# Thefefe/orbit

Measured on NVIDIA B200. Metric: Gmeshlets culled/s (C2: 10k entities / 2M meshlets, 1920x1080, two-pass occlusion, steady-state frame), higher is better.
Workload: dtype f32

## Files before the change

### orbit_b200/csrc/meshlet_cull.cu

```cuda
#include "params.cuh"

namespace orbit {

constexpr int kMcWarps = 8;
constexpr int kMcThreads = kMcWarps * 32;
constexpr int kMvStride = 20;
constexpr uint32_t kNone = 0xFFFFFFFFu;

struct ItemTest {
    Sphere s;
    bool pre_visible;
};

template <int kProj>
__device__ __forceinline__ ItemTest test_item(const OrbitCullInfo& ci, const float4 c0, const float4 c1, const float4 c2, const float4 c3,
                                              const float scale, const float cx, const float cy, const float cz, const float r_model,
                                              const uint32_t cone) {
    ItemTest out;
    float px = add(add(add(mul(c0.x, cx), mul(c1.x, cy)), mul(c2.x, cz)), c3.x);
    float py = add(add(add(mul(c0.y, cx), mul(c1.y, cy)), mul(c2.y, cz)), c3.y);
    float pz = add(add(add(mul(c0.z, cx), mul(c1.z, cy)), mul(c2.z, cz)), c3.z);
    const float pw = add(add(add(mul(c0.w, cx), mul(c1.w, cy)), mul(c2.w, cz)), c3.w);
    if (pw != 1.0f) { px = fdiv(px, pw); py = fdiv(py, pw); pz = fdiv(pz, pw); }
    Sphere& s = out.s;
    s.x = px; s.y = py; s.z = pz;
    s.r_model = r_model; s.s = scale;
    s.r = mul(s.r_model, scale);
    const float nr = -s.r;
    bool visible = true;
    const uint32_t n = ci.cull_plane_count;
    if (n == 5u) {
#pragma unroll
        for (uint32_t i = 0; i < 5u; ++i) {
            const float d = add(dot3(ci.cull_planes[i][0], ci.cull_planes[i][1], ci.cull_planes[i][2], px, py, pz), ci.cull_planes[i][3]);
            visible = visible && (d > nr);
        }
    } else {
#pragma unroll 1
        for (uint32_t i = 0; i < n; ++i) {
            const float d = add(dot3(ci.cull_planes[i][0], ci.cull_planes[i][1], ci.cull_planes[i][2], px, py, pz), ci.cull_planes[i][3]);
            visible = visible && (d > nr);
        }
    }
    {
        const float K = 0.007874015718698502f;
        const float kx = mul((float)(int)(int8_t)(cone & 0xFFu), K);
        const float ky = mul((float)(int)(int8_t)((cone >> 8) & 0xFFu), K);
        const float kz = mul((float)(int)(int8_t)((cone >> 16) & 0xFFu), K);
        const float cutoff = mul((float)((int)cone >> 24), K);
        const float axx = add(add(add(mul(c0.x, kx), mul(c1.x, ky)), mul(c2.x, kz)), mul(c3.x, 0.0f));
        const float axy = add(add(add(mul(c0.y, kx), mul(c1.y, ky)), mul(c2.y, kz)), mul(c3.y, 0.0f));
        const float axz = add(add(add(mul(c0.z, kx), mul(c1.z, ky)), mul(c2.z, kz)), mul(c3.z, 0.0f));
        const uint32_t proj = kProj >= 0 ? (uint32_t)kProj : ci.projection_type;
        if (proj == 0u) {
            const float lhs = dot3(px, py, pz, axx, axy, axz);
            const float len = fsqrt(dot3(px, py, pz, px, py, pz));
            visible = visible && !(lhs >= fma_(cutoff, len, s.r));
        } else if (proj == 1u) {
            const float camx = sub(px, 0.0f), camy = sub(py, 0.0f), camz = sub(pz, -1.0f);
            const float qx = sub(px, camx), qy = sub(py, camy), qz = sub(pz, camz);
            const float lhs = dot3(qx, qy, qz, axx, axy, axz);
            const float len = fsqrt(dot3(qx, qy, qz, qx, qy, qz));
            visible = visible && !(lhs >= fma_(cutoff, len, s.r));
        }
    }
    out.pre_visible = visible;
    return out;
}

__device__ __forceinline__ bool draw_rule(const OrbitCullInfo& ci, const MeshletCullParams& p, bool visible, bool vib, bool pass2,
                                          uint32_t packed) {
    if (!visible) return false;
    const uint32_t material_index = packed & 0xFFFFu;
    const uint32_t alpha = __ldg(reinterpret_cast<const uint32_t*>(
        p.materials + (size_t)material_index * ORBIT_MATERIAL_STRIDE_BYTES + ORBIT_MATERIAL_ALPHA_MODE_OFFSET));
    bool should_draw = (shl1(alpha) & ci.alpha_mode_flags) != 0u;
    if (pass2 && (shl1(alpha) & ci.noskip_alpha_mode) == 0u) should_draw = !vib;
    return should_draw;
}

__device__ __forceinline__ void store_command(uint32_t* __restrict__ dst, uint32_t vertex_offset, uint32_t data_offset, uint32_t packed,
                                              uint32_t entity, uint32_t meshlet_index) {
    dst[0] = (packed >> 24) * 3u;
    dst[1] = 1u;
    dst[2] = (data_offset + ((packed >> 16) & 0xFFu)) * 4u;
    dst[3] = data_offset;
    dst[4] = entity;
    dst[5] = vertex_offset;
    dst[6] = meshlet_index;
}

constexpr uint32_t kMaxChunks = 2048u;
__device__ __forceinline__ uint32_t chunk_shift_of(uint32_t nrec) {
    const uint32_t per = (nrec + kMaxChunks - 1u) / kMaxChunks;
    const uint32_t sh = per <= 1u ? 0u : 32u - (uint32_t)__clz((int)(per - 1u));
    return max(5u, sh);
}

__device__ __forceinline__ uint32_t smem_addr(const void* p) { return (uint32_t)__cvta_generic_to_shared(p); }
__device__ __forceinline__ void cp_async_16_stream(uint32_t dst, const void* src, uint64_t policy) {
    asm volatile("cp.async.cg.shared.global.L2::cache_hint [%0], [%1], 16, %2;" ::"r"(dst), "l"(src), "l"(policy) : "memory");
}
__device__ __forceinline__ void cp_async_16(uint32_t dst, const void* src) {
    asm volatile("cp.async.cg.shared.global [%0], [%1], 16;" ::"r"(dst), "l"(src) : "memory");
}
__device__ __forceinline__ void cp_async_4(uint32_t dst, const void* src) {
    asm volatile("cp.async.ca.shared.global [%0], [%1], 4;" ::"r"(dst), "l"(src) : "memory");
}
__device__ __forceinline__ void cp_async_commit() { asm volatile("cp.async.commit_group;" ::: "memory"); }
__device__ __forceinline__ void cp_async_wait_all() { asm volatile("cp.async.wait_group 0;" ::: "memory"); }
__device__ __forceinline__ uint64_t l2_evict_first_policy() {
    uint64_t pol;
    asm volatile("createpolicy.fractional.L2::evict_first.b64 %0, 1.0;" : "=l"(pol));
    return pol;
}
__device__ __forceinline__ void sts32(uint32_t addr, uint32_t v) { asm volatile("st.shared.u32 [%0], %1;" ::"r"(addr), "r"(v) : "memory"); }
__device__ __forceinline__ uint32_t lds32(uint32_t addr) { uint32_t v; asm volatile("ld.shared.u32 %0, [%1];" : "=r"(v) : "r"(addr) : "memory"); return v; }
__device__ __forceinline__ uint4 lds128(uint32_t addr) {
    uint4 v;
    asm volatile("ld.shared.v4.u32 {%0, %1, %2, %3}, [%4];" : "=r"(v.x), "=r"(v.y), "=r"(v.z), "=r"(v.w) : "r"(addr) : "memory");
    return v;
}

struct PkConsts { float2 one, mone; };
ORBIT_DEV float2 pk(float a, float b) { return make_float2(a, b); }
ORBIT_DEV float2 pmul(float2 a, float2 b) { return __fmul2_rn(a, b); }
ORBIT_DEV float2 pmuls(float2 a, float s) { return __fmul2_rn(a, make_float2(s, s)); }
ORBIT_DEV float2 pfma(float2 a, float2 b, float2 c) { return __ffma2_rn(a, b, c); }
ORBIT_DEV float2 padd(const PkConsts& k, float2 a, float2 b) { return __ffma2_rn(a, k.one, b); }
ORBIT_DEV float2 psub(const PkConsts& k, float2 a, float2 b) { return __ffma2_rn(b, k.mone, a); }
ORBIT_DEV float2 pneg(const PkConsts& k, float2 a) { return __fmul2_rn(a, k.mone); }
ORBIT_DEV float2 pdot3(const PkConsts& k, float2 ax, float2 ay, float2 az, float2 bx, float2 by, float2 bz) {
    return padd(k, padd(k, pmul(ax, bx), pmul(ay, by)), pmul(az, bz));
}
ORBIT_DEV float2 psqrt(float2 a) { return make_float2(fsqrt(a.x), fsqrt(a.y)); }
ORBIT_DEV float2 pdiv(float2 a, float2 b) { return make_float2(fdiv(a.x, b.x), fdiv(a.y, b.y)); }

struct ItemXY { float2 pxy; float pz, r; bool pre_visible; };
ORBIT_DEV float2 lo2(const float4 v) { return make_float2(v.x, v.y); }
ORBIT_DEV float2 hi2(const float4 v) { return make_float2(v.z, v.w); }

template <int kProj>
__device__ __forceinline__ ItemXY test_item_xy(const OrbitCullInfo& ci, const MeshletCullParams& p, const PkConsts& k, const float4 c0, const float4 c1,
                                              const float4 c2, const float4 c3, const float scale, const float cx, const float cy, const float cz,
                                              const float r_model, const uint32_t cone) {
    ItemXY out;
    float2 pxy = padd(k, padd(k, padd(k, pmuls(lo2(c0), cx), pmuls(lo2(c1), cy)), pmuls(lo2(c2), cz)), lo2(c3));
    const float2 pzw = padd(k, padd(k, padd(k, pmuls(hi2(c0), cx), pmuls(hi2(c1), cy)), pmuls(hi2(c2), cz)), hi2(c3));
    float pz = pzw.x;
    if (pzw.y != 1.0f) { pxy.x = fdiv(pxy.x, pzw.y); pxy.y = fdiv(pxy.y, pzw.y); pz = fdiv(pz, pzw.y); }
    const float r = mul(r_model, scale);
    out.pxy = pxy; out.pz = pz; out.r = r;
// ... 63 lines not shown
        const float2 nrc1 = pmul(nr, c1), rc1 = pmul(r, c1);
        const float2 sxc0 = pmul(sx, c0), sxc1 = pmul(sx, c1), syd0 = pmul(sy, d0), syc1 = pmul(sy, c1);
        const float2 minx0 = padd(k, sxc0, nrc1), minx1 = padd(k, pmul(r, c0), sxc1);
        const float2 maxx0 = padd(k, sxc0, rc1), maxx1 = padd(k, pmul(nr, c0), sxc1);
        const float2 miny0 = padd(k, syd0, nrc1), miny1 = padd(k, pmul(r, d0), syc1);
        const float2 maxy0 = padd(k, syd0, rc1), maxy1 = padd(k, pmul(nr, d0), syc1);
        const float2 a0 = pmuls(pdiv(minx0, minx1), P00), a1 = pmuls(pdiv(miny0, miny1), P11);
        const float2 a2 = pmuls(pdiv(maxx0, maxx1), P00), a3 = pmuls(pdiv(maxy0, maxy1), P11);
        const float2 h = pk(0.5f, 0.5f), nh = pk(-0.5f, -0.5f);
        ax = pfma(a0, h, h); ay = pfma(a3, nh, h);
        az = pfma(a2, h, h); aw = pfma(a1, nh, h);
        depth = pdiv(pk(ci.z_near, ci.z_near), pfma(pneg(k, r_model), s, zp));
    } else if (proj == 1u) {
        const float sr = ci.p00_or_width_recip_x2;
        const float2 ctrx = pmuls(x, sr), ctry = pmuls(y, sr);
        const float2 box = pmuls(r, sr);
        const float2 one = pk(1.0f, 1.0f), mone = pk(-1.0f, -1.0f);
        float2 b0 = pfma(box, mone, ctrx), b1 = pfma(box, mone, ctry);
        float2 b2 = pfma(box, one, ctrx), b3 = pfma(box, one, ctry);
        b0 = pk(fminf(fmaxf(b0.x, -1.0f), 1.0f), fminf(fmaxf(b0.y, -1.0f), 1.0f));
        b1 = pk(fminf(fmaxf(b1.x, -1.0f), 1.0f), fminf(fmaxf(b1.y, -1.0f), 1.0f));
        b2 = pk(fminf(fmaxf(b2.x, -1.0f), 1.0f), fminf(fmaxf(b2.y, -1.0f), 1.0f));
        b3 = pk(fminf(fmaxf(b3.x, -1.0f), 1.0f), fminf(fmaxf(b3.y, -1.0f), 1.0f));
        const float2 h = pk(0.5f, 0.5f), nh = pk(-0.5f, -0.5f);
        ax = pfma(b0, h, h); ay = pfma(b1, nh, h);
        az = pfma(b2, h, h); aw = pfma(b3, nh, h);
        const float kk = fdiv(1.0f, sub(ci.z_far, ci.z_near));
        depth = pmuls(padd(k, pfma(r_model, s, z), pk(ci.z_far, ci.z_far)), kk);
    } else {
        return 3u;
    }
    const float2 W = pmuls(psub(k, az, ax), (float)hz.width);
    const float2 H = pmuls(psub(k, aw, ay), (float)hz.height);
    const float2 u = pmuls(padd(k, ax, az), 0.5f), v = pmuls(padd(k, ay, aw), 0.5f);
    uint32_t vis = 0u;
    {
        const uint32_t lvl = hiz_level(fmaxf(W.x, H.x), hz.levels);
        const float sampled = hiz_sample(hz, hiz_lw, hiz_lh, lvl, u.x, v.x);
        if (!cull_a || depth.x >= sampled) vis |= 1u;
    }
    {
        const uint32_t lvl = hiz_level(fmaxf(W.y, H.y), hz.levels);
        const float sampled = hiz_sample(hz, hiz_lw, hiz_lh, lvl, u.y, v.y);
        if (!cull_b || depth.y >= sampled) vis |= 2u;
    }
    return vis;
}
struct RecordWords { uint32_t ent, moff, cnt, vo; };

template <int kProj>
__device__ __forceinline__ uint32_t drain_candidates(const MeshletCullParams& p, const PkConsts& k, const uint32_t qbase, const uint32_t ring_mask, const uint32_t qhead,
                                                  const uint32_t n, uint32_t* const chunk_counts, const uint32_t chunk_shift,
                                                  const uint32_t hiz_lw, const uint32_t hiz_lh, const uint32_t lane,
                                                  uint32_t* const main_chunk_counts, uint32_t& main_drawn_out) {
    const OrbitCullInfo& ci = p.cull;
    const uint32_t cs4 = (ring_mask + 1u) * 4u;
    uint32_t rec0 = 0xFFFFFFFFu, vo0 = 0u, vbits = 0u, lbits = 0u, mbits = 0u;
    uint32_t rec1 = 0xFFFFFFFFu, vo1 = 0u, vbit1 = 0u, lbit1 = 0u, mbit1 = 0u;
    if (2u * lane < n) {
        const uint32_t qa = qbase + ((qhead + 2u * lane) & ring_mask) * 4u;
        float2 cx, cy, cz, crm, cs;
        asm volatile("ld.shared.v2.f32 {%0, %1}, [%2];" : "=f"(cx.x), "=f"(cx.y) : "r"(qa) : "memory");
        asm volatile("ld.shared.v2.f32 {%0, %1}, [%2];" : "=f"(cy.x), "=f"(cy.y) : "r"(qa + 1u * cs4) : "memory");
        asm volatile("ld.shared.v2.f32 {%0, %1}, [%2];" : "=f"(cz.x), "=f"(cz.y) : "r"(qa + 2u * cs4) : "memory");
        asm volatile("ld.shared.v2.f32 {%0, %1}, [%2];" : "=f"(crm.x), "=f"(crm.y) : "r"(qa + 3u * cs4) : "memory");
        asm volatile("ld.shared.v2.f32 {%0, %1}, [%2];" : "=f"(cs.x), "=f"(cs.y) : "r"(qa + 4u * cs4) : "memory");
        uint32_t vis = occlusion_pair<kProj>(ci, k, cx, cy, cz, crm, cs, p.hiz, hiz_lw, hiz_lh);
        if (2u * lane + 1u >= n) vis &= 1u;
#pragma unroll
        for (uint32_t c = 0; c < 2u; ++c) {
            if ((vis >> c) & 1u) {
                const uint32_t rec = lds32(qa + 5u * cs4 + c * 4u), vo = lds32(qa + 6u * cs4 + c * 4u), id = lds32(qa + 7u * cs4 + c * 4u);
                const uint32_t bit = 1u << (id & 31u);
                const uint32_t abit = shl1(id >> 6);
                const bool draw = (abit & ci.noskip_alpha_mode) ? (abit & ci.alpha_mode_flags) != 0u : (id & 32u) == 0u;
                const bool mdraw = main_chunk_counts != nullptr && (abit & p.main_alpha_mode_flags) != 0u;
                if (rec0 == 0xFFFFFFFFu || rec == rec0) {
                    rec0 = rec; vo0 = vo; vbits |= bit; if (draw) lbits |= bit; if (mdraw) mbits |= bit;
                } else {
                    rec1 = rec; vo1 = vo; vbit1 = bit; if (draw) lbit1 = bit; if (mdraw) mbit1 = bit;
                }
            }
        }
    }
    __syncwarp();
    uint32_t drawn = 0u;
    uint32_t todo = __ballot_sync(0xFFFFFFFFu, vbits != 0u);
    if (todo != 0u) {
        const bool any_late = __any_sync(0xFFFFFFFFu, (lbits | lbit1) != 0u);
        while (todo != 0u) {
            const uint32_t key = __shfl_sync(0xFFFFFFFFu, rec0, __ffs((int)todo) - 1);
            const bool mine = vbits != 0u && rec0 == key;
            const uint32_t same = __ballot_sync(0xFFFFFFFFu, mine);
            const uint32_t v = __reduce_or_sync(0xFFFFFFFFu, mine ? vbits : 0u);
            const uint32_t l = any_late ? __reduce_or_sync(0xFFFFFFFFu, mine ? lbits : 0u) : 0u;
            const uint32_t m = main_chunk_counts != nullptr ? __reduce_or_sync(0xFFFFFFFFu, mine ? mbits : 0u) : 0u;
            if (lane == (uint32_t)(__ffs((int)same) - 1)) {
                atomicOr(p.meshlet_visibility + vo0, v);
                if (l != 0u) { atomicOr(reinterpret_cast<uint32_t*>(p.draw_masks + rec0), l); atomicAdd(chunk_counts + (rec0 >> chunk_shift), (uint32_t)__popc(l)); }
                if (m != 0u) { atomicOr(reinterpret_cast<uint32_t*>(p.main_masks + rec0), m); atomicAdd(main_chunk_counts + (rec0 >> chunk_shift), (uint32_t)__popc(m)); }
            }
            todo &= ~same;
        }
        if (vbit1 != 0u) {
            atomicOr(p.meshlet_visibility + vo1, vbit1);
            if (lbit1 != 0u) { atomicOr(reinterpret_cast<uint32_t*>(p.draw_masks + rec1), lbit1); atomicAdd(chunk_counts + (rec1 >> chunk_shift), 1u); }
            if (mbit1 != 0u) { atomicOr(reinterpret_cast<uint32_t*>(p.main_masks + rec1), mbit1); atomicAdd(main_chunk_counts + (rec1 >> chunk_shift), 1u); }
        }
        __syncwarp();
        if (any_late) drawn = __reduce_add_sync(0xFFFFFFFFu, (uint32_t)__popc(lbits) + (lbit1 != 0u ? 1u : 0u));
        if (main_chunk_counts != nullptr) main_drawn_out += __reduce_add_sync(0xFFFFFFFFu, (uint32_t)__popc(mbits) + (mbit1 != 0u ? 1u : 0u));
    }
    return drawn;
}

__device__ __forceinline__ void mbar_init(uint32_t bar, uint32_t count) {
    asm volatile("mbarrier.init.shared::cta.b64 [%0], %1;" ::"r"(bar), "r"(count) : "memory");
}
__device__ __forceinline__ void mbar_fence_init() { asm volatile("fence.mbarrier_init.release.cluster;" ::: "memory"); }
__device__ __forceinline__ void mbar_arrive_expect_tx(uint32_t bar, uint32_t bytes) {
    asm volatile("mbarrier.arrive.expect_tx.shared::cta.b64 _, [%0], %1;" ::"r"(bar), "r"(bytes) : "memory");
}
__device__ __forceinline__ void mbar_arrive(uint32_t bar) {
    asm volatile("mbarrier.arrive.shared::cta.b64 _, [%0];" ::"r"(bar) : "memory");
}
__device__ __forceinline__ void mbar_wait(uint32_t bar, uint32_t parity) {
    asm volatile(
        "{\n"
        ".reg .pred P1;\n"
        "LAB_WAIT:\n"
        "mbarrier.try_wait.parity.shared::cta.b64 P1, [%0], %1;\n"
        "@P1 bra DONE;\n"
        "bra LAB_WAIT;\n"
        "DONE:\n"
        "}" ::"r"(bar), "r"(parity) : "memory");
}
__device__ __forceinline__ void tma_load_1d(uint32_t dst, const void* src, uint32_t bytes, uint32_t bar) {
    asm volatile("cp.async.bulk.shared::cluster.global.mbarrier::complete_tx::bytes [%0], [%1], %2, [%3];"
                 ::"r"(dst), "l"(src), "r"(bytes), "r"(bar) : "memory");
}

template <int R>
struct __align__(128) WarpSmem {
    uint4 meshlets[R * 64];
    float mv[R][kMvStride];
    float4 rows[R][4];
    uint32_t vis[4 * ((R + 3) / 4)];
    uint32_t q[8][128];
    unsigned long long bar;
};
constexpr uint32_t kRing = 128u;
#ifndef ORBIT_DIRECT_MIN_CTAS
#define ORBIT_DIRECT_MIN_CTAS 3
#endif
#ifndef ORBIT_DIRECT_WARPS
#define ORBIT_DIRECT_WARPS 8
#endif
constexpr int kDwWarps = ORBIT_DIRECT_WARPS;
constexpr int kDwThreads = kDwWarps * 32;

template <int R>
__device__ __forceinline__ void tile_model_view(const float4* rows, float* mv_base, uint32_t my_word, uint32_t lane,
                                                float v0, float v1, float v2, float v3) {
#pragma unroll
    for (int st = 0; st < R / 2; ++st) {
        const uint32_t half = lane >> 4, e = lane & 15u;
        const uint32_t cnt = __shfl_sync(0xFFFFFFFFu, my_word, (2 * st + half) * 4 + 2);
        if (cnt != 0u) {
            const float4 b = rows[(2 * st + half) * 4 + (e >> 2)];
            mv_base[(2 * st + half) * kMvStride + e] = add(add(add(mul(v0, b.x), mul(v1, b.y)), mul(v2, b.z)), mul(v3, b.w));
        }
    }
    __syncwarp();
    if (lane < (uint32_t)R) mv_base[lane * kMvStride + 16] = largest_scale(mv_base + lane * kMvStride);
    __syncwarp();
}

template <int R, bool kPass2, int kProj, bool kBatch>
__device__ __forceinline__ void meshlet_test_direct_body(const MeshletCullParams* views, uint32_t n_views) {
    static_assert(R == 2 || R == 4 || R == 8, "records per warp tile");
    static_assert(!(kBatch && kPass2), "batched views are pass 0");
    const MeshletCullParams& p = views[0];
    extern __shared__ __align__(128) unsigned char s_raw[];
    WarpSmem<R>* const all = reinterpret_cast<WarpSmem<R>*>(s_raw + 128);
    uint32_t* const s_next_tile = reinterpret_cast<uint32_t*>(s_raw);

    const uint32_t lane = threadIdx.x & 31u, warp = threadIdx.x >> 5;
    const uint32_t lt = (1u << lane) - 1u;
    WarpSmem<R>& ws = all[warp];
    const OrbitCullInfo& ci = p.cull;
    const PkConsts k = {p.pk_one, p.pk_mone};
    pdl_wait();
    ORBIT_TRACE_STAMP(p.scan.trace, 1, 0);
    if (threadIdx.x == 0) *s_next_tile = kDwWarps;
    __syncthreads();
    auto fetch_tile = [&]() -> uint32_t {
        uint32_t j = 0u;
        if (lane == 0u) j = atomicAdd(s_next_tile, 1u);
        j = __shfl_sync(0xFFFFFFFFu, j, 0);
        const uint64_t t = (uint64_t)blockIdx.x + (uint64_t)j * gridDim.x;
        return t < 0x7FFFFFFFull ? (uint32_t)t : 0x7FFFFFFFu;
    };
    uint32_t t_cur = blockIdx.x + warp * gridDim.x, t_next = fetch_tile(), t_next2 = fetch_tile();
    auto load_words = [&](uint32_t tile, uint64_t bound) -> uint32_t {
        uint32_t w = 0u;
        if (lane < 4u * R && (uint64_t)tile * R + (lane >> 2) < bound) w = __ldcg(p.dispatch_words + 3u + (size_t)tile * R * 4u + lane);
        return w;
    };
    uint32_t v_nrec = 0u, v_half = 0u, v_tile_end = 0u;
    if constexpr (kBatch) {
        if (lane < n_views) {
            v_nrec = (uint32_t)min((uint64_t)__ldcg(views[lane].dispatch_words), views[lane].capacity_records);
            v_half = __ldcg(views[lane].chunk_parity) & 1u;
            if (blockIdx.x == 0 && warp == 0u) views[lane].chunk_parity[1] = v_half;
        }
        v_tile_end = (v_nrec + R - 1) / R;
#pragma unroll
        for (int d = 1; d < 32; d <<= 1) {
            const uint32_t t = __shfl_up_sync(0xFFFFFFFFu, v_tile_end, d);
            if (lane >= (uint32_t)d) v_tile_end += t;
        }
    }
    struct ViewTile { uint32_t view, rec0, nrec; };
    auto locate = [&](uint32_t t) -> ViewTile {
        const uint32_t v = (uint32_t)__popc(__ballot_sync(0xFFFFFFFFu, lane < n_views && v_tile_end <= t));
        const uint32_t first = __shfl_sync(0xFFFFFFFFu, v_tile_end, (v - 1u) & 31u);
        return ViewTile{v, (t - (v ? first : 0u)) * R, __shfl_sync(0xFFFFFFFFu, v_nrec, v & 31u)};
    };
    auto load_view_words = [&](uint32_t tile) -> uint32_t {
        const ViewTile w = locate(tile);
        uint32_t x = 0u;
        if (lane < 4u * R && w.rec0 + (lane >> 2) < w.nrec) x = __ldcg(views[w.view].dispatch_words + 3u + (size_t)w.rec0 * 4u + lane);
        return x;
    };
    uint32_t cur_word = 0u, next_word = 0u, nrec = 0u;
    if constexpr (!kBatch) {
        cur_word = load_words(t_cur, p.capacity_records); next_word = load_words(t_next, p.capacity_records);
        nrec = __ldcg(p.dispatch_words);
        if ((uint64_t)nrec > p.capacity_records) nrec = (uint32_t)p.capacity_records;
    }
    ORBIT_TRACE_STAMP(p.scan.trace, 1, 1 + 0 * (nrec & 1u));
    uint32_t chunk_shift = chunk_shift_of(nrec);
    uint32_t half = 0u;
    if constexpr (!kBatch) {
        half = __ldcg(p.chunk_parity) & 1u;
        if (blockIdx.x == 0 && threadIdx.x == 0) p.chunk_parity[1] = half;
    }
    uint32_t* chunk_counts = p.chunk_counts + half * kMaxChunks;
    uint32_t* draw_total = p.draw_total + half;
    uint32_t* main_chunk_counts = nullptr;
    uint32_t main_total = 0u, mhalf = 0u;
    if (kPass2 && p.main_masks != nullptr) {
        mhalf = __ldcg(p.main_chunk_parity) & 1u;
        if (blockIdx.x == 0 && threadIdx.x == 0) p.main_chunk_parity[1] = mhalf;
        main_chunk_counts = p.main_chunk_counts + mhalf * kMaxChunks;
    }
    const uint32_t tiles_total = kBatch ? __shfl_sync(0xFFFFFFFFu, v_tile_end, 31) : (nrec + R - 1) / R;
    if constexpr (kBatch) {
        if (t_cur < tiles_total) cur_word = load_view_words(t_cur);
        if (t_next < tiles_total) next_word = load_view_words(t_next);
    }
    const uint32_t vrow_i = lane & 3u;
    float v0 = ci.view_matrix.m[0][vrow_i], v1 = ci.view_matrix.m[1][vrow_i];
    float v2 = ci.view_matrix.m[2][vrow_i], v3 = ci.view_matrix.m[3][vrow_i];
    uint32_t cur_view = kBatch ? 0xFFFFFFFFu : 0u;
    const uint32_t hiz_lw = 31u - (uint32_t)__clz((int)max(p.hiz.width, 1u)), hiz_lh = 31u - (uint32_t)__clz((int)max(p.hiz.height, 1u));
    float* const mv_base = &ws.mv[0][0];
    const uint32_t bar = smem_addr(&ws.bar);
    const uint32_t buf = smem_addr(&ws.meshlets[0]);
    const uint32_t qbase = smem_addr(&ws.q[0][0]);
    const uint32_t rows_s = smem_addr(&ws.rows[0][0]), vis_s = smem_addr(&ws.vis[0]);
    if (lane == 0u) { mbar_init(bar, R); mbar_fence_init(); }
    __syncwarp();
    uint32_t parity = 0u;

    auto issue_tma = [&](uint32_t words) {
        const uint32_t off = __shfl_sync(0xFFFFFFFFu, words, (lane * 4u + 1u) & 31u);
        const uint32_t cnt = __shfl_sync(0xFFFFFFFFu, words, (lane * 4u + 2u) & 31u);
        {
            const uint32_t rr = (lane >> 2) & (uint32_t)(R - 1);
            const uint32_t ent_r = __shfl_sync(0xFFFFFFFFu, words, rr * 4u + 0u), cnt_r = __shfl_sync(0xFFFFFFFFu, words, rr * 4u + 2u);
            if (lane < 4u * R && cnt_r != 0u) cp_async_16(rows_s + lane * 16u, p.entities + (size_t)ent_r * 8u + (lane & 3u));
            if (kPass2) {
                const uint32_t rv = lane & (uint32_t)(R - 1);
                const uint32_t vo_r = __shfl_sync(0xFFFFFFFFu, words, rv * 4u + 3u), cnt_v = __shfl_sync(0xFFFFFFFFu, words, rv * 4u + 2u);
                if (lane >= 16u && lane < 16u + (uint32_t)R && cnt_v != 0u) cp_async_4(vis_s + rv * 4u, p.meshlet_visibility + vo_r);
            }
            cp_async_commit();
        }
        if (lane < (uint32_t)R) {
            if (cnt != 0u) {
                const uint32_t bytes = min(cnt, 32u) * 32u;
                mbar_arrive_expect_tx(bar, bytes);
                tma_load_1d(buf + lane * 1024u, p.meshlets + 2u * (size_t)off, bytes, bar);
            } else {
                mbar_arrive(bar);
            }
        }
    };
    if constexpr (!kBatch) {
        if (!(lane < 4u * R && (uint64_t)t_cur * R + (lane >> 2) < (uint64_t)nrec)) cur_word = 0u;
        if (!(lane < 4u * R && (uint64_t)t_next * R + (lane >> 2) < (uint64_t)nrec)) next_word = 0u;
    }
    uint32_t warp_total = 0u;
#ifdef ORBIT_TRACE
    bool trace_first = true;
#endif
    uint32_t qhead = 0u, qn = 0u;
    if (t_cur < tiles_total) issue_tma(cur_word);
    bool final_pass = t_cur >= tiles_total;
    while (true) {
        uint32_t rec0 = t_cur * R;
        if constexpr (kBatch) {
            if (!final_pass) {
                const ViewTile w = locate(t_cur);
                rec0 = w.rec0; nrec = w.nrec;
                if (w.view != cur_view) {
                    if (lane == 0u && warp_total != 0u) atomicAdd(draw_total, warp_total);
                    warp_total = 0u;
                    cur_view = w.view;
                    const uint32_t h = __shfl_sync(0xFFFFFFFFu, v_half, cur_view);
                    chunk_shift = chunk_shift_of(nrec);
                    chunk_counts = views[cur_view].chunk_counts + h * kMaxChunks;
                    draw_total = views[cur_view].draw_total + h;
                    const OrbitCullInfo& cv = views[cur_view].cull;
                    v0 = cv.view_matrix.m[0][vrow_i]; v1 = cv.view_matrix.m[1][vrow_i];
                    v2 = cv.view_matrix.m[2][vrow_i]; v3 = cv.view_matrix.m[3][vrow_i];
                }
            }
        }
        const MeshletCullParams& pt = kBatch ? views[cur_view & (ORBIT_MAX_BATCH_VIEWS - 1)] : p;
        const uint32_t my_word = final_pass ? 0u : cur_word;
        uint32_t my_mask = 0u;
        uint32_t vw = 0u;
        if (!final_pass) {
            cur_word = next_word;
            if constexpr (kBatch) next_word = t_next2 < tiles_total ? load_view_words(t_next2) : 0u;
            else next_word = t_next2 < tiles_total ? load_words(t_next2, nrec) : 0u;
            if (kPass2) {
                const uint32_t ent = __shfl_sync(0xFFFFFFFFu, my_word, (lane * 4u + 0u) & 31u);
                const uint32_t mof = __shfl_sync(0xFFFFFFFFu, my_word, (lane * 4u + 1u) & 31u);
                const uint32_t my_cnt = __shfl_sync(0xFFFFFFFFu, my_word, (lane * 4u + 2u) & 31u);
                const uint32_t my_vo = __shfl_sync(0xFFFFFFFFu, my_word, (lane * 4u + 3u) & 31u);
                cp_async_wait_all();
                __syncwarp();
                if (lane < (uint32_t)R && my_cnt != 0u) {
                    vw = ws.vis[lane];
                    p.meshlet_visibility[my_vo] = 0u;
                }
                if (lane < (uint32_t)R && rec0 + lane < nrec) {
                    p.draw_masks[rec0 + lane] = make_uint4(0u, ent, mof, 1u);
                    if (main_chunk_counts != nullptr) p.main_masks[rec0 + lane] = make_uint4(0u, ent, mof, 1u);
                }
            } else {
                cp_async_wait_all();
                __syncwarp();
            }
            tile_model_view<R>(&ws.rows[0][0], mv_base, my_word, lane, v0, v1, v2, v3);
            mbar_wait(bar, parity);
            parity ^= 1u;
#ifdef ORBIT_TRACE
            if (p.scan.trace != nullptr && threadIdx.x == 0 && trace_first) { trace_first = false; ORBIT_TRACE_STAMP(p.scan.trace, 1, 2); }
#endif
        }
#pragma unroll 1
        for (uint32_t r = 0; r < (uint32_t)R; ++r) {
            const uint32_t cnt = __shfl_sync(0xFFFFFFFFu, my_word, r * 4u + 2u);
            if (cnt != 0u) {
                const float* mvr = mv_base + r * kMvStride;
                const float4 c0 = *reinterpret_cast<const float4*>(mvr), c1 = *reinterpret_cast<const float4*>(mvr + 4);
                const float4 c2 = *reinterpret_cast<const float4*>(mvr + 8), c3 = *reinterpret_cast<const float4*>(mvr + 12);
                const float scale = mvr[16];
                const bool in_rec = lane < cnt;
                const uint4 a = ws.meshlets[r * 64u + lane * 2u];
                const uint4 b = ws.meshlets[r * 64u + lane * 2u + 1u];
                uint32_t alpha = 32u;
                if (in_rec) alpha = __ldg(reinterpret_cast<const uint32_t*>(
                    p.materials + (size_t)(b.w & 0xFFFFu) * ORBIT_MATERIAL_STRIDE_BYTES + ORBIT_MATERIAL_ALPHA_MODE_OFFSET));
                const ItemXY t = test_item_xy<kProj>(pt.cull, pt, k, c0, c1, c2, c3, scale, __uint_as_float(a.x), __uint_as_float(a.y),
                                                     __uint_as_float(a.z), __uint_as_float(a.w), b.x);
                const bool pre = in_rec && t.pre_visible;
                if (!kPass2) {
                    const bool draw = pre && (shl1(alpha) & pt.cull.alpha_mode_flags) != 0u;
                    const uint32_t mask = __ballot_sync(0xFFFFFFFFu, draw);
                    if (lane == r) my_mask = mask;
                    const uint32_t ent_r = __shfl_sync(0xFFFFFFFFu, my_word, r * 4u);
                    if (draw && pt.cmd_side != nullptr) pt.cmd_side[(size_t)(rec0 + r) * 32u + lane] = make_uint4(b.y, b.z, b.w, ent_r);
                } else {
                    const uint32_t pre_mask = __ballot_sync(0xFFFFFFFFu, pre);
                    const uint32_t vwr = __shfl_sync(0xFFFFFFFFu, vw, r);
                    const uint32_t vo = __shfl_sync(0xFFFFFFFFu, my_word, r * 4u + 3u);
                    if (pre) {
                        const uint32_t id = lane | (((vwr >> lane) & 1u) << 5) | (min(alpha, 32u) << 6);
                        const uint32_t qa = qbase + ((qhead + qn + (uint32_t)__popc(pre_mask & lt)) & (kRing - 1u)) * 4u;
                        constexpr uint32_t cs4 = kRing * 4u;
                        sts32(qa, __float_as_uint(t.pxy.x)); sts32(qa + cs4, __float_as_uint(t.pxy.y)); sts32(qa + 2u * cs4, __float_as_uint(t.pz));
                        sts32(qa + 3u * cs4, a.w); sts32(qa + 4u * cs4, __float_as_uint(scale));
                        sts32(qa + 5u * cs4, rec0 + r); sts32(qa + 6u * cs4, vo); sts32(qa + 7u * cs4, id);
                    }
                    qn += (uint32_t)__popc(pre_mask);
                }
            }
            if (kPass2 && (qn >= 64u || (final_pass && qn != 0u))) {
                const uint32_t n = min(qn, 64u);
                __syncwarp();
                warp_total += drain_candidates<kProj>(p, k, qbase, kRing - 1u, qhead, n, chunk_counts, chunk_shift, hiz_lw, hiz_lh, lane,
                                                      main_chunk_counts, main_total);
                qhead = (qhead + n) & (kRing - 1u);
                qn -= n;
            }
        }
        if (final_pass) break;
        __syncwarp();
        if (t_next < tiles_total) issue_tma(cur_word);
        if (!kPass2) {
            const uint32_t ent = __shfl_sync(0xFFFFFFFFu, my_word, (lane * 4u + 0u) & 31u);
            const uint32_t mof = __shfl_sync(0xFFFFFFFFu, my_word, (lane * 4u + 1u) & 31u);
            if (lane < (uint32_t)R && rec0 + lane < nrec) pt.draw_masks[rec0 + lane] = make_uint4(my_mask, ent, mof, pt.cmd_side != nullptr ? 0u : 1u);
            const uint32_t tile_total = __reduce_add_sync(0xFFFFFFFFu, __popc(my_mask));
            if (lane == 0u && tile_total != 0u) atomicAdd(chunk_counts + (rec0 >> chunk_shift), tile_total);
            warp_total += tile_total;
        }
        t_cur = t_next; t_next = t_next2;
        t_next2 = t_next2 < tiles_total ? fetch_tile() : 0x7FFFFFFFu;
        final_pass = t_cur >= tiles_total;
    }
    ORBIT_TRACE_STAMP(p.scan.trace, 1, 3);
    pdl_launch_dependents();
    if (lane == 0u && warp_total != 0u) atomicAdd(draw_total, warp_total);
    if (kPass2 && lane == 0u && main_total != 0u) atomicAdd(p.main_draw_total + mhalf, main_total);
#ifdef ORBIT_TRACE
    __syncthreads();
    ORBIT_TRACE_STAMP(p.scan.trace, 1, 4);
#endif
}

template <int R, bool kPass2, int kProj>
__global__ void __launch_bounds__(kDwThreads, ORBIT_DIRECT_MIN_CTAS) meshlet_test_direct_kernel(const __grid_constant__ MeshletCullParams p) {
    meshlet_test_direct_body<R, kPass2, kProj, false>(&p, 1u);
}

template <int R, int kProj>
__global__ void __launch_bounds__(kDwThreads, ORBIT_DIRECT_MIN_CTAS) meshlet_test_views_kernel(const __grid_constant__ MeshletViewsParams pv) {
    meshlet_test_direct_body<R, false, kProj, true>(pv.view, pv.n_views);
}

template <int R>
struct __align__(16) PackedCtaSmem {
    float mv[kMcWarps][R][kMvStride];
    uint32_t words[kMcWarps][R * 4];
    uint32_t mask[kMcWarps][R];
    uint32_t queue[kMcWarps * R * 32];
    uint32_t qcount[2];
};

template <int R>
struct PackedPrefetch {
    float4 b[R / 2];
    uint32_t vw;
};

template <int R>
__device__ __forceinline__ PackedPrefetch<R> packed_issue_loads(const MeshletCullParams& p, uint32_t words, uint32_t lane) {
    PackedPrefetch<R> f;
    const uint32_t my_cnt = __shfl_sync(0xFFFFFFFFu, words, (lane * 4u + 2u) & 31u);
    const uint32_t my_vo = __shfl_sync(0xFFFFFFFFu, words, (lane * 4u + 3u) & 31u);
    f.vw = 0u;
    if (lane < (uint32_t)R && my_cnt != 0u) f.vw = __ldcg(p.meshlet_visibility + my_vo) & (my_cnt >= 32u ? 0xFFFFFFFFu : ((1u << my_cnt) - 1u));
#pragma unroll
    for (int st = 0; st < R / 2; ++st) {
        const uint32_t half = lane >> 4, e = lane & 15u;
        const uint32_t ent = __shfl_sync(0xFFFFFFFFu, words, (2 * st + half) * 4 + 0);
        const uint32_t cnt = __shfl_sync(0xFFFFFFFFu, words, (2 * st + half) * 4 + 2);
        f.b[st] = make_float4(0.f, 0.f, 0.f, 0.f);
        if (cnt != 0u) f.b[st] = __ldg(p.entities + (size_t)ent * 8u + (e >> 2));
    }
    return f;
}

template <int R>
__device__ __forceinline__ void packed_finish_model_view(const PackedPrefetch<R>& f, float* mv_base, uint32_t lane,
                                                         float v0, float v1, float v2, float v3) {
#pragma unroll
    for (int st = 0; st < R / 2; ++st) {
        const uint32_t half = lane >> 4, e = lane & 15u;
        const float4 b = f.b[st];
// ... 470 lines not shown
    const uint32_t nrec = (uint32_t)min((uint64_t)s_region[p.n_regions], p.capacity_records);
    const uint32_t chunk_shift = chunk_shift_of(nrec);
    const uint32_t half = __ldcg(p.chunk_parity) & 1u;
    if (blockIdx.x == 0 && threadIdx.x == 0) { p.chunk_parity[1] = half; header_out[0] = nrec; header_out[1] = 1u; header_out[2] = 1u; }
    uint32_t* const chunk_counts = p.chunk_counts + half * kMaxChunks;
    const uint32_t lane = threadIdx.x & 31u;
    uint32_t mine = 0u;
    for (uint64_t base = ((uint64_t)blockIdx.x * blockDim.x + threadIdx.x) & ~31ull; base < nrec; base += (uint64_t)gridDim.x * blockDim.x) {
        const uint32_t r = (uint32_t)base + lane;
        uint32_t pc = 0u;
        if (r < nrec) {
            uint32_t k = 0u;
            while (k + 1u < p.n_regions && r >= s_region[k + 1u]) ++k;
            pc = (uint32_t)__popc(__ldcg(reinterpret_cast<const uint32_t*>(p.draw_masks + (size_t)k * p.region_stride + (r - s_region[k]))));
        }
        const uint32_t s = __reduce_add_sync(0xFFFFFFFFu, pc);
        if (lane == 0u && s != 0u) { atomicAdd(chunk_counts + (uint32_t)(base >> chunk_shift), s); mine += s; }
    }
    if (mine != 0u) atomicAdd(p.draw_total + half, mine);
}

cudaError_t launch_record_masks_put(const uint4* src, const uint32_t* dispatch_words, uint4* dst_region, uint32_t* dst_count, uint64_t capacity,
                                    int grid, cudaStream_t s) {
    record_masks_put_kernel<<<grid, 256, 0, s>>>(src, dispatch_words, dst_region, dst_count, capacity);
    return cudaGetLastError();
}

cudaError_t launch_draws_from_masks(const MeshletCullParams& p, uint32_t* header, int grid, int emit_grid, cudaStream_t s) {
    record_masks_recount_kernel<<<grid, 256, 0, s>>>(p, header);
    cudaError_t e = cudaGetLastError();
    if (e != cudaSuccess) return e;
    return launch_kernel(meshlet_emit_kernel, dim3(emit_grid), dim3(kEmitWarps * 32), 0, s, p);
}

struct TestVariant { bool packed; bool pass2; int proj; };
static TestVariant variant_of(const OrbitCullInfo& ci) {
    const bool mocc = ci.meshlet_visibility_buffer != ORBIT_NO_BUFFER;
    TestVariant v;
    v.packed = ci.occlusion_pass == 1u && mocc;
    v.pass2 = ci.occlusion_pass == 2u && mocc;
    v.proj = ci.projection_type <= 1u ? (int)ci.projection_type : -1;
    return v;
}

#ifndef ORBIT_TILE_RECORDS
#define ORBIT_TILE_RECORDS 4
#endif
constexpr int kTileR = ORBIT_TILE_RECORDS;
#ifndef ORBIT_PACKED_RECORDS
#define ORBIT_PACKED_RECORDS 8
#endif
constexpr int kPackedR = ORBIT_PACKED_RECORDS;
static constexpr size_t direct_smem_bytes() { return 128u + sizeof(WarpSmem<kTileR>) * kDwWarps; }

template <bool kPass2, int kProj>
static cudaError_t launch_stream(const MeshletCullParams& p, int grid, cudaStream_t stream, int* occupancy) {
    if (occupancy) {
        cudaOccupancyMaxActiveBlocksPerMultiprocessor(occupancy, meshlet_test_direct_kernel<kTileR, kPass2, kProj>, kDwThreads, direct_smem_bytes());
        return cudaSuccess;
    }
    return launch_kernel(meshlet_test_direct_kernel<kTileR, kPass2, kProj>, dim3(grid), dim3(kDwThreads), direct_smem_bytes(), stream, p);
}

cudaError_t meshlet_cull_configure_device() {
    cudaError_t e;
#define ORBIT_SET(kp2, proj) \
    e = cudaFuncSetAttribute(meshlet_test_direct_kernel<kTileR, kp2, proj>, cudaFuncAttributeMaxDynamicSharedMemorySize, (int)direct_smem_bytes()); \
    if (e != cudaSuccess) return e;
    ORBIT_SET(false, 0) ORBIT_SET(false, 1) ORBIT_SET(false, -1) ORBIT_SET(true, 0) ORBIT_SET(true, 1) ORBIT_SET(true, -1)
#undef ORBIT_SET
#define ORBIT_SET(proj) \
    e = cudaFuncSetAttribute(meshlet_test_views_kernel<kTileR, proj>, cudaFuncAttributeMaxDynamicSharedMemorySize, (int)direct_smem_bytes()); \
    if (e != cudaSuccess) return e;
    ORBIT_SET(0) ORBIT_SET(1) ORBIT_SET(-1)
#undef ORBIT_SET
    return cudaSuccess;
}

static cudaError_t launch_test(const MeshletCullParams& p, int grid, cudaStream_t stream, int* occupancy) {
    const TestVariant v = variant_of(p.cull);
    if (v.packed) {
        if (occupancy) { cudaOccupancyMaxActiveBlocksPerMultiprocessor(occupancy, meshlet_test_packed_kernel<kPackedR>, kMcThreads, 0); return cudaSuccess; }
        return launch_kernel(meshlet_test_packed_kernel<kPackedR>, dim3(grid), dim3(kMcThreads), 0, stream, p);
    }
    if (v.pass2) {
        if (v.proj == 0) return launch_stream<true, 0>(p, grid, stream, occupancy);
        if (v.proj == 1) return launch_stream<true, 1>(p, grid, stream, occupancy);
        return launch_stream<true, -1>(p, grid, stream, occupancy);
    }
    if (v.proj == 0) return launch_stream<false, 0>(p, grid, stream, occupancy);
    if (v.proj == 1) return launch_stream<false, 1>(p, grid, stream, occupancy);
    return launch_stream<false, -1>(p, grid, stream, occupancy);
}

int meshlet_cull_variant_index(const OrbitCullInfo& ci) {
    const TestVariant v = variant_of(ci);
    return v.packed ? 0 : 1 + (v.pass2 ? 3 : 0) + (v.proj + 1);
}

int meshlet_cull_max_ctas_per_sm(const MeshletCullParams& p) {
    int n = 0;
    launch_test(p, 0, nullptr, &n);
    return n;
}

cudaError_t launch_meshlet_emit(const MeshletCullParams& p, int emit_grid, cudaStream_t stream) {
    return launch_kernel(meshlet_emit_kernel, dim3(emit_grid), dim3(kEmitWarps * 32), 0, stream, p);
}
cudaError_t launch_meshlet_emit_pair(const MeshletCullParams& a, const MeshletCullParams& b, int emit_grid, cudaStream_t stream) {
    EmitPair pp;
    pp.list[0] = a; pp.list[1] = b;
    return launch_kernel(meshlet_emit_pair_kernel, dim3(emit_grid, 2), dim3(kEmitWarps * 32), 0, stream, pp);
}

cudaError_t launch_meshlet_cull(const MeshletCullParams& p, int grid, int emit_grid, cudaStream_t stream) {
    if (grid > 0) {
        cudaError_t e = launch_test(p, grid, stream, nullptr);
        if (e != cudaSuccess) return e;
    }
    if (emit_grid > 0) return launch_kernel(meshlet_emit_kernel, dim3(emit_grid), dim3(kEmitWarps * 32), 0, stream, p);
// ... 38 lines not shown
```

Measured before the change: 24.82.

## Share pass-2 candidate queue across warps via CTA-wide ring buffer

Replaces the per-warp 128-entry occlusion candidate queue in the pass-2 direct kernel with a single 1024-entry ring shared by the whole CTA. Warps reserve slots atomically, publish batch counts with acquire/release fences, and any warp may claim a full 64-candidate batch to drain. A last-producer handoff flushes the leftover partial batch. The aim is fuller drain batches and less tail imbalance where warps end with partial queues. In exchange it adds shared-memory atomics, spin-wait with nanosleep, and fairly involved ordering logic that carries deadlock and race risk.

Result: slower. 21.19 (median of 6 runs) (-14.6%).

```diff
diff --git a/orbit_b200/csrc/meshlet_cull.cu b/orbit_b200/csrc/meshlet_cull.cu
--- a/orbit_b200/csrc/meshlet_cull.cu
+++ b/orbit_b200/csrc/meshlet_cull.cu
@@ -1,3 +1,5 @@
+#include <type_traits>
+
 #include "params.cuh"
 
 namespace orbit {
@@ -98,6 +100,12 @@
 }
 
 __device__ __forceinline__ uint32_t smem_addr(const void* p) { return (uint32_t)__cvta_generic_to_shared(p); }
+__device__ __forceinline__ void fence_acq_rel_cta() { asm volatile("fence.acq_rel.cta;" ::: "memory"); }
+__device__ __forceinline__ uint32_t ld_acquire_shared(const uint32_t* p) {
+    uint32_t v;
+    asm volatile("ld.acquire.cta.shared::cta.u32 %0, [%1];" : "=r"(v) : "r"(smem_addr(p)) : "memory");
+    return v;
+}
 __device__ __forceinline__ void cp_async_16_stream(uint32_t dst, const void* src, uint64_t policy) {
     asm volatile("cp.async.cg.shared.global.L2::cache_hint [%0], [%1], 16, %2;" ::"r"(dst), "l"(src), "l"(policy) : "memory");
 }
@@ -267,7 +275,7 @@
 __device__ __forceinline__ uint32_t drain_candidates(const MeshletCullParams& p, const PkConsts& k, const uint32_t qbase, const uint32_t ring_mask, const uint32_t qhead,
                                                   const uint32_t n, uint32_t* const chunk_counts, const uint32_t chunk_shift,
                                                   const uint32_t hiz_lw, const uint32_t hiz_lh, const uint32_t lane,
-                                                  uint32_t* const main_chunk_counts, uint32_t& main_drawn_out) {
+                                                  uint32_t* const main_chunk_counts, uint32_t& main_drawn_out, uint32_t* const release_slot) {
     const OrbitCullInfo& ci = p.cull;
     const uint32_t cs4 = (ring_mask + 1u) * 4u;
     uint32_t rec0 = 0xFFFFFFFFu, vo0 = 0u, vbits = 0u, lbits = 0u, mbits = 0u;
@@ -299,6 +307,7 @@
         }
     }
     __syncwarp();
+    if (release_slot != nullptr && lane == 0u) { fence_acq_rel_cta(); atomicAdd(release_slot, ring_mask + 1u - 64u); }
     uint32_t drawn = 0u;
     uint32_t todo = __ballot_sync(0xFFFFFFFFu, vbits != 0u);
     if (todo != 0u) {
@@ -364,7 +373,31 @@
     uint32_t q[8][128];
     unsigned long long bar;
 };
-constexpr uint32_t kRing = 128u;
+template <int R>
+struct __align__(128) TileSmem {
+    uint4 meshlets[R * 64];
+    float mv[R][kMvStride];
+    float4 rows[R][4];
+    uint32_t vis[4 * ((R + 3) / 4)];
+    unsigned long long bar;
+};
+constexpr uint32_t kCtaRing = 1024u;
+#ifndef ORBIT_RING_SLEEP_MIN
+#define ORBIT_RING_SLEEP_MIN 32
+#endif
+#ifndef ORBIT_RING_SLEEP_MAX
+#define ORBIT_RING_SLEEP_MAX 32
+#endif
+constexpr uint32_t kRingBatches = kCtaRing / 64u;
+struct CtaRingHeader {
+    uint32_t next_tile;
+    uint32_t reserved;
+    uint32_t claimed;
+    uint32_t producers_done;
+    uint32_t batch[kRingBatches];
+    unsigned long long last_drain;
+};
+static_assert(sizeof(CtaRingHeader) <= 128, "ring header");
 #ifndef ORBIT_DIRECT_MIN_CTAS
 #define ORBIT_DIRECT_MIN_CTAS 3
 #endif
@@ -397,17 +430,26 @@
     static_assert(!(kBatch && kPass2), "batched views are pass 0");
     const MeshletCullParams& p = views[0];
     extern __shared__ __align__(128) unsigned char s_raw[];
-    WarpSmem<R>* const all = reinterpret_cast<WarpSmem<R>*>(s_raw + 128);
+    using WS = std::conditional_t<kPass2, TileSmem<R>, WarpSmem<R>>;
+    WS* const all = reinterpret_cast<WS*>(s_raw + 128 + (kPass2 ? 8u * kCtaRing * 4u : 0u));
     uint32_t* const s_next_tile = reinterpret_cast<uint32_t*>(s_raw);
+    CtaRingHeader* const rh = reinterpret_cast<CtaRingHeader*>(s_raw);
 
     const uint32_t lane = threadIdx.x & 31u, warp = threadIdx.x >> 5;
     const uint32_t lt = (1u << lane) - 1u;
-    WarpSmem<R>& ws = all[warp];
+    WS& ws = all[warp];
     const OrbitCullInfo& ci = p.cull;
     const PkConsts k = {p.pk_one, p.pk_mone};
     pdl_wait();
     ORBIT_TRACE_STAMP(p.scan.trace, 1, 0);
     if (threadIdx.x == 0) *s_next_tile = kDwWarps;
+    if constexpr (kPass2) {
+        if (threadIdx.x == 0) { rh->reserved = 0u; rh->claimed = 0u; rh->producers_done = 0u; }
+        if (threadIdx.x < kRingBatches) rh->batch[threadIdx.x] = 0u;
+#ifdef ORBIT_TRACE
+        if (threadIdx.x == 0) rh->last_drain = 0ull;
+#endif
+    }
     __syncthreads();
     auto fetch_tile = [&]() -> uint32_t {
         uint32_t j = 0u;
@@ -483,7 +525,7 @@
     float* const mv_base = &ws.mv[0][0];
     const uint32_t bar = smem_addr(&ws.bar);
     const uint32_t buf = smem_addr(&ws.meshlets[0]);
-    const uint32_t qbase = smem_addr(&ws.q[0][0]);
+    const uint32_t qbase = smem_addr(s_raw + 128);
     const uint32_t rows_s = smem_addr(&ws.rows[0][0]), vis_s = smem_addr(&ws.vis[0]);
     if (lane == 0u) { mbar_init(bar, R); mbar_fence_init(); }
     __syncwarp();
@@ -521,10 +563,16 @@
 #ifdef ORBIT_TRACE
     bool trace_first = true;
 #endif
-    uint32_t qhead = 0u, qn = 0u;
     if (t_cur < tiles_total) issue_tma(cur_word);
     bool final_pass = t_cur >= tiles_total;
+    bool last_producer = false;
     while (true) {
+        if constexpr (kPass2) {
+            if (final_pass) {
+                if (lane == 0u) { fence_acq_rel_cta(); last_producer = atomicAdd(&rh->producers_done, 1u) == (uint32_t)kDwWarps - 1u; }
+                ORBIT_TRACE_STAMP(p.scan.trace, 1, 3);
+            }
+        }
         uint32_t rec0 = t_cur * R;
         if constexpr (kBatch) {
             if (!final_pass) {
@@ -581,6 +629,8 @@
 #pragma unroll 1
         for (uint32_t r = 0; r < (uint32_t)R; ++r) {
             const uint32_t cnt = __shfl_sync(0xFFFFFFFFu, my_word, r * 4u + 2u);
+            uint32_t q_run = 0u, q_first = 0u, q_slot = kNone;
+            uint32_t qw[8];
             if (cnt != 0u) {
                 const float* mvr = mv_base + r * kMvStride;
                 const float4 c0 = *reinterpret_cast<const float4*>(mvr), c1 = *reinterpret_cast<const float4*>(mvr + 4);
@@ -606,23 +656,80 @@
                     const uint32_t vwr = __shfl_sync(0xFFFFFFFFu, vw, r);
                     const uint32_t vo = __shfl_sync(0xFFFFFFFFu, my_word, r * 4u + 3u);
                     if (pre) {
+                        q_slot = (uint32_t)__popc(pre_mask & lt);
                         const uint32_t id = lane | (((vwr >> lane) & 1u) << 5) | (min(alpha, 32u) << 6);
-                        const uint32_t qa = qbase + ((qhead + qn + (uint32_t)__popc(pre_mask & lt)) & (kRing - 1u)) * 4u;
-                        constexpr uint32_t cs4 = kRing * 4u;
-                        sts32(qa, __float_as_uint(t.pxy.x)); sts32(qa + cs4, __float_as_uint(t.pxy.y)); sts32(qa + 2u * cs4, __float_as_uint(t.pz));
-                        sts32(qa + 3u * cs4, a.w); sts32(qa + 4u * cs4, __float_as_uint(scale));
-                        sts32(qa + 5u * cs4, rec0 + r); sts32(qa + 6u * cs4, vo); sts32(qa + 7u * cs4, id);
+                        qw[0] = __float_as_uint(t.pxy.x); qw[1] = __float_as_uint(t.pxy.y); qw[2] = __float_as_uint(t.pz);
+                        qw[3] = a.w; qw[4] = __float_as_uint(scale); qw[5] = rec0 + r; qw[6] = vo; qw[7] = id;
                     }
-                    qn += (uint32_t)__popc(pre_mask);
+                    q_run = (uint32_t)__popc(pre_mask);
+                    if (q_run != 0u) {
+                        uint32_t e = 0u;
+                        if (lane == 0u) e = atomicAdd(&rh->reserved, q_run);
+                        q_first = __shfl_sync(0xFFFFFFFFu, e, 0);
+                    }
                 }
             }
-            if (kPass2 && (qn >= 64u || (final_pass && qn != 0u))) {
-                const uint32_t n = min(qn, 64u);
-                __syncwarp();
-                warp_total += drain_candidates<kProj>(p, k, qbase, kRing - 1u, qhead, n, chunk_counts, chunk_shift, hiz_lw, hiz_lh, lane,
-                                                      main_chunk_counts, main_total);
-                qhead = (qhead + n) & (kRing - 1u);
-                qn -= n;
+            if constexpr (kPass2) {
+                uint32_t nap = ORBIT_RING_SLEEP_MIN;
+                while (true) {
+                    if (q_run != 0u) {
+                        uint32_t room = 0u;
+                        if (lane == 0u) {
+                            const uint32_t e1 = q_first + q_run - 1u;
+                            room = (int)(ld_acquire_shared(&rh->batch[(q_first >> 6) % kRingBatches]) - (q_first & ~(kCtaRing - 1u))) >= 0 &&
+                                   (int)(ld_acquire_shared(&rh->batch[(e1 >> 6) % kRingBatches]) - (e1 & ~(kCtaRing - 1u))) >= 0;
+                        }
+                        if (__shfl_sync(0xFFFFFFFFu, room, 0) != 0u) {
+                            __syncwarp();
+                            if (q_slot != kNone) {
+                                const uint32_t qa = qbase + ((q_first + q_slot) % kCtaRing) * 4u;
+#pragma unroll
+                                for (int w = 0; w < 8; ++w) sts32(qa + (uint32_t)w * kCtaRing * 4u, qw[w]);
+                            }
+                            __syncwarp();
+                            if (lane == 0u) {
+                                fence_acq_rel_cta();
+                                const uint32_t n0 = min(q_run, 64u - (q_first & 63u));
+                                atomicAdd(&rh->batch[(q_first >> 6) % kRingBatches], n0);
+                                if (q_run > n0) atomicAdd(&rh->batch[((q_first + q_run - 1u) >> 6) % kRingBatches], q_run - n0);
+                            }
+                            q_run = 0u;
+                        }
+                    }
+                    constexpr uint32_t kCtaDone = 0x80000000u;
+                    uint32_t job = 0u;
+                    if (lane == 0u) {
+                        const uint32_t ce = ld_acquire_shared(&rh->claimed);
+                        if (ld_acquire_shared(&rh->batch[(ce >> 6) % kRingBatches]) == (ce & ~(kCtaRing - 1u)) + 64u) {
+                            if (atomicCAS(&rh->claimed, ce, ce + 64u) == ce) job = (64u << 16) | (ce % kCtaRing);
+                        } else if (last_producer) {
+                            last_producer = false;
+                            (void)ld_acquire_shared(&rh->producers_done);
+                            const uint32_t tot = ld_acquire_shared(&rh->reserved);
+                            if ((tot & 63u) != 0u) job = ((tot & 63u) << 16) | (tot % kCtaRing & ~63u);
+                        } else if (final_pass && ld_acquire_shared(&rh->producers_done) == (uint32_t)kDwWarps) {
+                            if (ld_acquire_shared(&rh->reserved) - ld_acquire_shared(&rh->claimed) < 64u) job = kCtaDone;
+                        }
+                    }
+                    job = __shfl_sync(0xFFFFFFFFu, job, 0);
+                    if (job != 0u && job != kCtaDone) {
+                        const uint32_t n = job >> 16, head = job & 0xFFFFu;
+                        __syncwarp();
+                        warp_total += drain_candidates<kProj>(p, k, qbase, kCtaRing - 1u, head, n, chunk_counts, chunk_shift, hiz_lw, hiz_lh,
+                                                              lane, main_chunk_counts, main_total, n == 64u ? &rh->batch[head / 64u] : nullptr);
+#ifdef ORBIT_TRACE
+                        if (lane == 0u && p.scan.trace != nullptr) atomicMax(&rh->last_drain, trace_time());
+#endif
+                        continue;
+                    }
+                    if (q_run == 0u && (!final_pass || job == kCtaDone)) break;
+#ifdef ORBIT_RING_NO_WAIT
+                    if (q_run == 0u && final_pass && __shfl_sync(0xFFFFFFFFu, (uint32_t)(ld_acquire_shared(&rh->producers_done) < (uint32_t)kDwWarps), 0)) break;
+#endif
+                    __nanosleep(nap);
+                    nap = min(2u * nap, (uint32_t)ORBIT_RING_SLEEP_MAX);
+                }
+                if (final_pass) break;
             }
         }
         if (final_pass) break;
@@ -640,13 +747,14 @@
         t_next2 = t_next2 < tiles_total ? fetch_tile() : 0x7FFFFFFFu;
         final_pass = t_cur >= tiles_total;
     }
-    ORBIT_TRACE_STAMP(p.scan.trace, 1, 3);
+    if constexpr (!kPass2) ORBIT_TRACE_STAMP(p.scan.trace, 1, 3);
     pdl_launch_dependents();
     if (lane == 0u && warp_total != 0u) atomicAdd(draw_total, warp_total);
     if (kPass2 && lane == 0u && main_total != 0u) atomicAdd(p.main_draw_total + mhalf, main_total);
 #ifdef ORBIT_TRACE
     __syncthreads();
     ORBIT_TRACE_STAMP(p.scan.trace, 1, 4);
+    if constexpr (kPass2) ORBIT_TRACE_VALUE(p.scan.trace, 5, rh->last_drain);
 #endif
 }
 
@@ -1223,20 +1331,24 @@
 #endif
 constexpr int kPackedR = ORBIT_PACKED_RECORDS;
 static constexpr size_t direct_smem_bytes() { return 128u + sizeof(WarpSmem<kTileR>) * kDwWarps; }
+static constexpr size_t direct_ring_smem_bytes() { return 128u + 8u * kCtaRing * 4u + sizeof(TileSmem<kTileR>) * kDwWarps; }
+static_assert(direct_ring_smem_bytes() <= direct_smem_bytes(), "the CTA ring must not grow the pass-2 kernel's shared memory");
+template <bool kPass2>
+static constexpr size_t direct_kernel_smem_bytes() { return kPass2 ? direct_ring_smem_bytes() : direct_smem_bytes(); }
 
 template <bool kPass2, int kProj>
 static cudaError_t launch_stream(const MeshletCullParams& p, int grid, cudaStream_t stream, int* occupancy) {
     if (occupancy) {
-        cudaOccupancyMaxActiveBlocksPerMultiprocessor(occupancy, meshlet_test_direct_kernel<kTileR, kPass2, kProj>, kDwThreads, direct_smem_bytes());
+        cudaOccupancyMaxActiveBlocksPerMultiprocessor(occupancy, meshlet_test_direct_kernel<kTileR, kPass2, kProj>, kDwThreads, direct_kernel_smem_bytes<kPass2>());
         return cudaSuccess;
     }
-    return launch_kernel(meshlet_test_direct_kernel<kTileR, kPass2, kProj>, dim3(grid), dim3(kDwThreads), direct_smem_bytes(), stream, p);
+    return launch_kernel(meshlet_test_direct_kernel<kTileR, kPass2, kProj>, dim3(grid), dim3(kDwThreads), direct_kernel_smem_bytes<kPass2>(), stream, p);
 }
 
 cudaError_t meshlet_cull_configure_device() {
     cudaError_t e;
 #define ORBIT_SET(kp2, proj) \
-    e = cudaFuncSetAttribute(meshlet_test_direct_kernel<kTileR, kp2, proj>, cudaFuncAttributeMaxDynamicSharedMemorySize, (int)direct_smem_bytes()); \
+    e = cudaFuncSetAttribute(meshlet_test_direct_kernel<kTileR, kp2, proj>, cudaFuncAttributeMaxDynamicSharedMemorySize, (int)direct_kernel_smem_bytes<kp2>()); \
     if (e != cudaSuccess) return e;
     ORBIT_SET(false, 0) ORBIT_SET(false, 1) ORBIT_SET(false, -1) ORBIT_SET(true, 0) ORBIT_SET(true, 1) ORBIT_SET(true, -1)
 #undef ORBIT_SET
```
